# facebookresearch/vsc2022

Hardware: AMD Instinct MI355X
Metric: query-videos localized/sec @ 512-d SSCD (higher is better)
Workload: dtype fp32 results; int8 / fp16 MFMA pre-filters; 1 GPU; BASELINE configs[3]: full pipeline incl. score normalisation + TN localisation, 40000 query videos split over 1 GPU(s), 2000000 reference + 2000000 noise frames; query_videos_per_gpu=40000, query_frames_per_gpu=1000000, ref_frames=2000000, dim=512, global_k=48000000, candidates=1000000, pairs_localized=200000, matches=446939, hits=48000000, score_normalisation_in_step=True, parallelism=single GPU

## Files before the change

vsc2022_amd/csrc/tn.hip:

```cpp
#include <cfloat>

#include "kernels.h"

namespace vscmi {

typedef float f32x16 __attribute__((ext_vector_type(16)));
typedef float f32x4 __attribute__((ext_vector_type(4)));


template <class IDX>
struct TnStateT {
    int lq, lr, top, ms, n_nodes, sink, sink_q, sink_r;
    unsigned top_magic;
    float min_sim;
    const IDX* tidx;
    const float* tsim;
    const IDX* ilo;
    const IDX* ihi;
};

template <class IDX>
__device__ __forceinline__ int tn_div_top(const TnStateT<IDX>& g, int x) {
    return g.top == 1 ? x : (int)__umulhi((unsigned)x, g.top_magic);
}
template <class IDX>
__device__ __forceinline__ int tn_node_q(const TnStateT<IDX>& g, int v) { return v == 0 ? -1 : tn_div_top(g, v - 1); }
template <class IDX>
__device__ __forceinline__ int tn_node_k(const TnStateT<IDX>& g, int v) { return (v - 1) - tn_div_top(g, v - 1) * g.top; }
template <class IDX>
__device__ __forceinline__ int tn_node_r(const TnStateT<IDX>& g, int v) { return v == 0 ? -1 : g.tidx[v - 1]; }

template <class IDX>
__device__ __forceinline__ bool tn_edge_ok(const TnStateT<IDX>& g, int qi, int a, int d, int b) {
    const int qj = qi + d;
    const int ra = g.tidx[qi * g.top + a], rb = g.tidx[qj * g.top + b];
    const int rd = rb - ra;
    if (!(rd > 0 && rd < g.ms)) return false;
    const int lo = g.ilo[qi * g.ms + d], hi = g.ihi[qi * g.ms + d];
    if (lo <= hi && !(hi < ra || lo > rb)) return false;
    return g.tsim[qj * g.top + b] >= g.min_sim;
}

template <class IDX>
__device__ __forceinline__ bool tn_sink_ok(const TnStateT<IDX>& g, int u) {
    if (u == g.sink) return false;
    const int qu = tn_node_q(g, u), ru = tn_node_r(g, u);
    return g.sink_q > qu && g.sink_r > ru && g.sink_q - qu <= g.ms && g.sink_r - ru <= g.ms;
}

template <class IDX>
__device__ __forceinline__ int tn_edge_bit(const TnStateT<IDX>& g, int qi, int a, int d, int b) {
    return (((qi + d) * g.top + b) * g.ms + d) * g.top + a;
}

__device__ __forceinline__ unsigned long long first_max_key(float v, int o) {
    const float vz = v + 0.0f;
    const unsigned b = __float_as_uint(vz);
    unsigned hi = (b & 0x80000000u) ? ~b : (b | 0x80000000u);
    hi = (vz != vz) ? 1u : hi;
    const unsigned long long k = ((unsigned long long)hi << 32) | (unsigned)(0x7fffffff - o);
    return o < 0 ? 0ull : k;
}
__device__ __forceinline__ void first_max_unkey(unsigned long long k, float& v, int& o) {
    const unsigned hi = (unsigned)(k >> 32);
    const float kv = __uint_as_float((hi & 0x80000000u) ? (hi & 0x7fffffffu) : ~hi);
    v = k ? kv : 0.0f;
    o = k ? 0x7fffffff - (int)(unsigned)k : -1;
}
template <int FIRST_OFF>
__device__ __forceinline__ void first_max_reduce(float& v, int& o) {
    unsigned long long k = first_max_key(v, o);
#pragma unroll
    for (int off = FIRST_OFF; off >= 1; off >>= 1) {
        const unsigned long long ok = __shfl_xor(k, off);
        k = ok > k ? ok : k;
    }
    first_max_unkey(k, v, o);
}
__device__ __forceinline__ void wave_first_max(float& v, int& o) { first_max_reduce<32>(v, o); }
__device__ __forceinline__ void half_first_max(float& v, int& o) { first_max_reduce<16>(v, o); }


#ifdef VSC_TN_PROFILE
__device__ unsigned long long tn_prof[8];
#define TN_T0() unsigned long long t_prof = __builtin_readcyclecounter()
#define TN_T(k)                                                                          \
    do {                                                                                 \
        const unsigned long long t_now = __builtin_readcyclecounter();                   \
        if (threadIdx.x == 0) atomicAdd(&tn_prof[k], t_now - t_prof);                    \
        t_prof = t_now;                                                                  \
    } while (0)
#else
#define TN_T0() do {} while (0)
#define TN_T(k) do {} while (0)
#endif

template <class IDX, bool GSTATE>
__global__ __launch_bounds__(64) void tn_pair_kernel(TnPairArgs a) {
    extern __shared__ __attribute__((aligned(16))) char smem_lds[];
    char* const smem = GSTATE ? a.state + (int64_t)blockIdx.x * a.state_bytes : smem_lds;
    const int lane = threadIdx.x;
    if ((int)blockIdx.x >= a.n_work) return;
    const int pidx = a.work[blockIdx.x];
    int64_t qrow0 = 0, rrow0 = 0;
    int lq, lr;
    if (a.sims_in) {
        lq = a.sims_lq[pidx];
        lr = a.sims_lr[pidx];
    } else {
        const int qv = a.pair_q[pidx], rv = a.pair_r[pidx];
        qrow0 = a.q_off[qv];
        rrow0 = a.r_off[rv];
        lq = (int)(a.q_off[qv + 1] - qrow0);
        lr = (int)(a.r_off[rv + 1] - rrow0);
    }
    const int ms = a.prm.tn_max_step > 1 ? a.prm.tn_max_step : 1;
    const int top_cap = a.prm.tn_top_k;
    const int top = top_cap < lr ? top_cap : lr;
    int32_t* o_nbox = a.out_nbox + pidx;
    int32_t* o_boxes = a.out_boxes + (int64_t)pidx * VSC_TN_MAX_BOXES * 4;
    float* o_bmax = a.out_boxmax + (int64_t)pidx * VSC_TN_MAX_BOXES;
    if (lq <= 0 || top <= 0) {
        if (lane == 0) *o_nbox = 0;
        return;
    }
    const int n_nodes = 1 + lq * top;

    size_t off = 0;
    IDX* tidx = reinterpret_cast<IDX*>(smem + off);
    off += (size_t)a.max_lq * top_cap * sizeof(IDX);
    off = (off + 15) & ~(size_t)15;
    float* tsim = reinterpret_cast<float*>(smem + off);
    off += (size_t)a.max_lq * top_cap * 4;
    IDX* ilo = reinterpret_cast<IDX*>(smem + off);
    off += (size_t)a.max_lq * ms * sizeof(IDX);
    IDX* ihi = reinterpret_cast<IDX*>(smem + off);
    off += (size_t)a.max_lq * ms * sizeof(IDX);
    off = (off + 15) & ~(size_t)15;
    unsigned int* zero = reinterpret_cast<unsigned int*>(smem + off);
    const int zero_words = (lq * top * ms * top + 31) / 32;
    off += ((size_t)a.max_lq * top_cap * ms * top_cap + 31) / 32 * 4;
    off = (off + 15) & ~(size_t)15;
    float* dist = reinterpret_cast<float*>(smem + off);
    off += (size_t)(1 + a.max_lq * top_cap) * 4;
    IDX* par = reinterpret_cast<IDX*>(smem + off);
    off += (size_t)(1 + a.max_lq * top_cap) * sizeof(IDX);
    IDX* order = reinterpret_cast<IDX*>(smem + off);
    off += (size_t)(1 + a.max_lq * top_cap) * sizeof(IDX);
    IDX* indeg = reinterpret_cast<IDX*>(smem + off);
    off += (size_t)(1 + a.max_lq * top_cap) * sizeof(IDX);
    off = (off + 15) & ~(size_t)15;
    int* boxes = reinterpret_cast<int*>(smem + off);
    off += (size_t)VSC_TN_MAX_BOXES * 16;
    unsigned long long* okmask = reinterpret_cast<unsigned long long*>(smem + off);
    off += (size_t)a.max_lq * ((top_cap + 1) / 2) * 8;
    off = (off + 63) & ~(size_t)63;
    float* sims;
    if (a.sims_in) sims = const_cast<float*>(a.sims_in) + a.sims_off[pidx];
    else if ((int64_t)lq * lr <= a.lds_tile_floats) sims = reinterpret_cast<float*>(smem + off);
    else sims = a.slab + (int64_t)blockIdx.x * a.slab_floats;

    TN_T0();
    if (!a.sims_in) {
        const int hi = lane >> 5, l31 = lane & 31;
        const int nkg = a.dpad / 8;
        for (int qb = 0; qb < lq; qb += 32)
            for (int rb = 0; rb < lr; rb += 64) {
                const bool two = rb + 32 < lr;
                const float* ap = a.qfeat + (qrow0 + qb + l31) * a.dpad + hi * 4;
                const float* bp0 = a.rfeat + (rrow0 + rb + l31) * a.dpad + hi * 4;
                const float* bp1 = bp0 + (two ? 32 * (int64_t)a.dpad : 0);
                f32x16 acc0, acc1;
#pragma unroll
                for (int r = 0; r < 16; ++r) acc0[r] = acc1[r] = 0.0f;
                if (two) {
#pragma unroll 4
                    for (int g = 0; g < nkg; ++g) {
                        const f32x4 av = *reinterpret_cast<const f32x4*>(ap + g * 8);
                        const f32x4 bv0 = *reinterpret_cast<const f32x4*>(bp0 + g * 8);
                        const f32x4 bv1 = *reinterpret_cast<const f32x4*>(bp1 + g * 8);
#pragma unroll
                        for (int s = 0; s < 4; ++s) {
                            acc0 = __builtin_amdgcn_mfma_f32_32x32x2f32(av[s], bv0[s], acc0, 0, 0, 0);
                            acc1 = __builtin_amdgcn_mfma_f32_32x32x2f32(av[s], bv1[s], acc1, 0, 0, 0);
                        }
                    }
                } else {
#pragma unroll 4
                    for (int g = 0; g < nkg; ++g) {
                        const f32x4 av = *reinterpret_cast<const f32x4*>(ap + g * 8);
                        const f32x4 bv = *reinterpret_cast<const f32x4*>(bp0 + g * 8);
#pragma unroll
                        for (int s = 0; s < 4; ++s)
                            acc0 = __builtin_amdgcn_mfma_f32_32x32x2f32(av[s], bv[s], acc0, 0, 0, 0);
                    }
                }
#pragma unroll
                for (int r = 0; r < 16; ++r) {
                    const int q = qb + (r & 3) + 8 * (r >> 2) + 4 * hi;
                    const int rr = rb + l31;
                    if (q < lq && rr < lr) sims[(int64_t)q * lr + rr] = acc0[r] + a.bias;
                    if (two && q < lq && rr + 32 < lr) sims[(int64_t)q * lr + rr + 32] = acc1[r] + a.bias;
                }
            }
    }
    for (int x = lane; x < zero_words; x += 64) zero[x] = 0;
    __threadfence_block();
    __syncthreads();
    TN_T(0);

    if (top_cap <= 8 && (lq >= 16 || lr <= 128)) {
        for (int q0 = 0; q0 < lq; q0 += 64) {
            const int q = q0 + lane;
            float ts[8];
            int ti[8];
#pragma unroll
            for (int e = 0; e < 8; ++e) {
                ts[e] = -INFINITY;
                ti[e] = -1;
            }
            if (q < lq) {
                const float* row = sims + (int64_t)q * lr;
                for (int r = 0; r < lr; ++r) {
                    const float sv = row[r];
                    if (!(sv > ts[7]) && ti[7] >= 0) continue;
#pragma unroll
                    for (int e = 7; e >= 1; --e) {
                        const bool empty_above = ti[e - 1] < 0;
                        const bool up = empty_above || sv > ts[e - 1];
                        const bool here = !up && (ti[e] < 0 || sv > ts[e]);
                        ts[e] = up ? ts[e - 1] : (here ? sv : ts[e]);
                        ti[e] = up ? ti[e - 1] : (here ? r : ti[e]);
                    }
                    if (ti[0] < 0 || sv > ts[0]) {
                        ts[0] = sv;
                        ti[0] = r;
                    }
                }
#pragma unroll
                for (int e = 0; e < 8; ++e)
                    if (e < top) {
                        tidx[q * top + e] = (IDX)ti[e];
                        tsim[q * top + e] = ts[e];
                    }
            }
        }
    } else {
        for (int q = 0; q < lq; ++q) {
            const float* row = sims + (int64_t)q * lr;
            float prev_s = INFINITY;
            int prev_r = -1;
            for (int e = 0; e < top; ++e) {
                float bs = 0.0f;
                int br = -1;
                for (int r = lane; r < lr; r += 64) {
                    const float s = row[r];
                    const bool after = (s < prev_s) || (s == prev_s && r > prev_r);
                    if (after && (br < 0 || s > bs)) {
                        bs = s;
                        br = r;
                    }
                }
                wave_first_max(bs, br);
                if (lane == 0) {
                    tidx[q * top + e] = (IDX)br;
                    tsim[q * top + e] = bs;
                }
                prev_s = bs;
                prev_r = br;
            }
        }
    }
    __syncthreads();

    TnStateT<IDX> g;
    g.lq = lq; g.lr = lr; g.top = top; g.ms = ms; g.n_nodes = n_nodes; g.sink = n_nodes - 1;
    g.sink_q = lq - 1;
    g.sink_r = tidx[(lq - 1) * top + top - 1];
    g.min_sim = a.prm.min_sim;
    g.top_magic = (unsigned)((0x100000000ull + (unsigned)top - 1u) / (unsigned)top);
    g.tidx = tidx; g.tsim = tsim; g.ilo = ilo; g.ihi = ihi;

    for (int qi = lane; qi < lq; qi += 64) {
        int lo = 1, hi = 0;
        for (int d = 1; d < ms; ++d) {
            ilo[qi * ms + d] = (IDX)lo;
            ihi[qi * ms + d] = (IDX)hi;
            if (qi + d >= lq) continue;
            int nlo = lo, nhi = hi;
            for (int b = 0; b < top; ++b) {
                bool any = false;
                for (int aa = 0; aa < top && !any; ++aa) any = tn_edge_ok(g, qi, aa, d, b);
                if (any) {
                    const int rb = tidx[(qi + d) * top + b];
                    if (nlo > nhi) nlo = nhi = rb;
                    else {
                        nlo = rb < nlo ? rb : nlo;
                        nhi = rb > nhi ? rb : nhi;
                    }
                }
            }
            lo = nlo;
            hi = nhi;
        }
    }
    __syncthreads();

    TN_T(1);
    const int P = (ms - 1) * top;
    int nbox = 0;
    bool have_order = false;
    const int hw_half = lane >> 5, hw_o = lane & 31;
    const int hw_d = ms - 1 - hw_o / top, hw_aa = hw_o % top;
    const int hw_bit_off = hw_d * top + hw_aa + hw_half * ms * top;
    const int hw_pred_off = 1 + hw_aa - hw_d * top;
    for (int it = 0; it <= a.prm.max_path; ++it) {
        if (lane == 0) {
            dist[0] = 0.0f;
            par[0] = 0;
        }
        __syncthreads();
        for (int qj = 0; qj < lq; ++qj) {
            int b_first = 0;
            if (P <= 32) {
                const int half = hw_half, o = hw_o, d = hw_d, aa = hw_aa;
                const int qi = qj - d;
                const int pred = qj * top + hw_pred_off;
                for (int b0 = 0; b0 < top; b0 += 2) {
                    const int b = b0 + half;
                    const int v = 1 + qj * top + b;
                    const bool mine = b < top && v != g.sink;
                    float c = 0.0f;
                    int oo = -1;
                    const int mslot = qj * ((top + 1) / 2) + (b0 >> 1);
                    bool ok;
                    if (it == 0) {
                        ok = mine && o < P && qi >= 0 && tn_edge_ok(g, qi, aa, d, b);
                        const unsigned long long m = __ballot(ok);
                        if (lane == 0) okmask[mslot] = m;
                    } else {
                        ok = (okmask[mslot] >> lane) & 1ull;
                    }
                    if (ok) {
                        const int bit = (qj * top + b0) * ms * top + hw_bit_off;
                        const bool z = (zero[bit >> 5] >> (bit & 31)) & 1u;
                        const float w = z ? 0.0f : tsim[qj * top + b];
                        c = dist[pred] + w;
                        oo = o;
                    }
                    half_first_max(c, oo);
                    const int pw = __shfl(pred, (lane & 32) | (oo < 0 ? 0 : oo));
                    if (mine && o == 0) {
                        if (oo < 0 || !(c >= 0.0f)) {
                            dist[v] = 0.0f;
                            par[v] = (IDX)v;
                        } else {
                            dist[v] = c;
                            par[v] = (IDX)pw;
                        }
                    }
                }
                b_first = (qj == lq - 1) ? top - 1 : top;
            }
            if (qj == lq - 1) TN_T(2);
            for (int b = b_first; b < top; ++b) {
                const int v = 1 + qj * top + b;
                const bool is_sink = (v == g.sink);
                float best = 0.0f;
                int arg = -1;
                for (int o0 = 0; o0 < P; o0 += 64) {
                    const int o = o0 + lane;
                    float c = 0.0f;
                    int oo = -1;
                    if (o < P) {
                        const int d = ms - 1 - o / top, aa = o % top;
                        const int qi = qj - d;
                        if (qi >= 0 && tn_edge_ok(g, qi, aa, d, b)) {
                            const int bit = tn_edge_bit(g, qi, aa, d, b);
                            const bool z = (zero[bit >> 5] >> (bit & 31)) & 1u;
                            const float w = (z || is_sink) ? 0.0f : tsim[qj * top + b];
                            c = dist[1 + qi * top + aa] + w;
                            oo = o;
                        }
                    }
                    wave_first_max(c, oo);
                    if (oo >= 0 && (arg < 0 || c > best)) {
                        best = c;
                        arg = oo;
                    }
                }
                int arg_node = -1;
                if (arg >= 0) arg_node = 1 + (qj - (ms - 1 - arg / top)) * top + arg % top;
                if (is_sink) {
                    for (int u0 = 0; u0 < n_nodes - 1; u0 += 64) {
                        const int u = u0 + lane;
                        float c = 0.0f;
                        int oo = -1;
                        if (u < n_nodes - 1 && tn_sink_ok(g, u)) {
                            bool regular = false;
                            if (u != 0) {
                                const int qi = tn_node_q(g, u), aa = tn_node_k(g, u);
                                const int d = qj - qi;
                                if (d >= 1 && d < ms) regular = tn_edge_ok(g, qi, aa, d, b);
                            }
                            if (!regular) {
                                c = dist[u] + 0.0f;
                                oo = u;
                            }
                        }
                        wave_first_max(c, oo);
                        if (oo >= 0 && (arg_node < 0 || c > best)) {
                            best = c;
                            arg_node = oo;
                        }
                    }
                }
                if (lane == 0) {
                    if (arg_node < 0 || !(best >= 0.0f)) {
                        dist[v] = 0.0f;
                        par[v] = (IDX)v;
                    } else {
                        dist[v] = best;
                        par[v] = (IDX)arg_node;
                    }
                }
            }
            __syncthreads();
        }

        TN_T(3);
        float mx = -FLT_MAX;
        int mxn = -1;
        for (int v = lane; v < n_nodes; v += 64) {
            const float dv = dist[v];
            if (mxn < 0 || dv > mx) {
                mx = dv;
                mxn = v;
            }
        }
        wave_first_max(mx, mxn);
        int ties = 0;
        for (int v = lane; v < n_nodes; v += 64) ties += (dist[v] == mx) ? 1 : 0;
#pragma unroll
        for (int off2 = 32; off2 >= 1; off2 >>= 1) ties += __shfl_xor(ties, off2);
        int vend = mxn;
        if (!(mx > 0.0f)) {
            vend = 0;
        } else if (ties > 1) {
            if (!have_order) {
                for (int v = lane; v < n_nodes; v += 64) {
                    int deg = 0;
                    if (v != 0) {
                        const int qj = tn_node_q(g, v), b = tn_node_k(g, v);
                        for (int d = 1; d < ms; ++d) {
                            const int qi = qj - d;
                            if (qi < 0) break;
                            for (int aa = 0; aa < top; ++aa) deg += tn_edge_ok(g, qi, aa, d, b) ? 1 : 0;
                        }
                        if (v == g.sink) {
                            for (int u = 0; u < n_nodes - 1; ++u) {
                                if (!tn_sink_ok(g, u)) continue;
                                bool regular = false;
                                if (u != 0) {
                                    const int qi = tn_node_q(g, u), aa = tn_node_k(g, u);
                                    const int d = qj - qi;
                                    if (d >= 1 && d < ms) regular = tn_edge_ok(g, qi, aa, d, b);
                                }
                                deg += regular ? 0 : 1;
                            }
                        }
                    }
                    indeg[v] = (IDX)deg;
                }
                __syncthreads();
                if (lane == 0) {
                    int head = 0, tail = 0;
                    for (int v = 0; v < n_nodes; ++v)
                        if (indeg[v] == 0) order[tail++] = (IDX)v;
                    while (head < tail) {
                        const int u = order[head++];
                        bool to_sink_regular = false;
                        if (u != 0) {
                            const int qi = tn_node_q(g, u), aa = tn_node_k(g, u);
                            for (int d = 1; d < ms && qi + d < lq; ++d)
                                for (int b = 0; b < top; ++b)
                                    if (tn_edge_ok(g, qi, aa, d, b)) {
                                        const int v = 1 + (qi + d) * top + b;
                                        if (v == g.sink) to_sink_regular = true;
                                        if (--indeg[v] == 0) order[tail++] = (IDX)v;
                                    }
                        }
                        if (!to_sink_regular && tn_sink_ok(g, u))
                            if (--indeg[g.sink] == 0) order[tail++] = (IDX)g.sink;
                    }
                }
                have_order = true;
                __syncthreads();
            }
            int bestpos = 0x7fffffff;
            for (int t = lane; t < n_nodes; t += 64)
                if (dist[order[t]] == mx && t < bestpos) bestpos = t;
#pragma unroll
            for (int off2 = 32; off2 >= 1; off2 >>= 1) {
                const int o2 = __shfl_xor(bestpos, off2);
                bestpos = o2 < bestpos ? o2 : bestpos;
            }
            vend = order[bestpos];
        }

        TN_T(4);
        int accepted = 0, stop = 0;
        int bq0 = 0, br0 = 0, bq1 = 0, br1 = 0;
        if (lane == 0) {
            int cnt = 0;
            for (int v = vend;;) {
                const int u = par[v];
                if (v != 0 && v != g.sink) ++cnt;
                if (u == v) break;
                if (u != 0) {
                    const int qi = tn_node_q(g, u), aa = tn_node_k(g, u);
                    const int qj = tn_node_q(g, v), b = tn_node_k(g, v);
                    const int d = qj - qi;
                    if (d >= 1 && d < ms && tn_edge_ok(g, qi, aa, d, b)) {
                        const int bit = tn_edge_bit(g, qi, aa, d, b);
                        zero[bit >> 5] |= 1u << (bit & 31);
                    }
                }
                v = u;
            }
            if (cnt == 0) {
                stop = 1;
            } else {
                int plen = 0;
                for (int v = vend;;) {
                    indeg[plen++] = (IDX)v;
                    if (par[v] == v) break;
                    v = par[v];
                }
                float score = 0.0f;
                int qmin = 0, qmax = 0, rmin = 0, rmax = 0, c2 = 0;
                for (int x = plen - 1; x >= 0; --x) {
                    const int v = indeg[x];
                    if (v == 0 || v == g.sink) continue;
                    const int q = tn_node_q(g, v), r = tn_node_r(g, v);
                    score += tsim[v - 1];
                    if (c2 == 0) {
                        qmin = qmax = q;
                        rmin = rmax = r;
                    } else {
                        qmin = q < qmin ? q : qmin;
                        qmax = q > qmax ? q : qmax;
                        rmin = r < rmin ? r : rmin;
                        rmax = r > rmax ? r : rmax;
                    }
                    ++c2;
                }
                if (!(score > 0.0f)) qmin = qmax = rmin = rmax = 0;
                const int dq = qmax - qmin, dr = rmax - rmin;
                const float ave = __fdiv_rn((float)(dr + dq), 2.0f);
                bool ok = (ave != 0.0f) && (__fdiv_rn(score, ave) > a.prm.min_sim) &&
                          ((dr < dq ? dr : dq) > a.prm.min_length);
                if (ok && nbox > 0) {
                    float mxi = -INFINITY;
                    for (int kx = 0; kx < nbox; ++kx) {
                        const int* o = boxes + 4 * kx;
                        const float lt0 = (float)(qmin > o[0] ? qmin : o[0]);
                        const float lt1 = (float)(rmin > o[1] ? rmin : o[1]);
                        const float rb0 = (float)(qmax < o[2] ? qmax : o[2]);
                        const float rb1 = (float)(rmax < o[3] ? rmax : o[3]);
                        const float w = rb0 - lt0 > 0.0f ? rb0 - lt0 : 0.0f;
                        const float h = rb1 - lt1 > 0.0f ? rb1 - lt1 : 0.0f;
                        const float inter = __fmul_rn(w, h);
                        const float aa2 = __fmul_rn((float)dq, (float)dr);
                        const float ab = __fmul_rn((float)(o[2] - o[0]), (float)(o[3] - o[1]));
                        const float iou = __fdiv_rn(inter, __fsub_rn(__fadd_rn(aa2, ab), inter));
                        mxi = iou > mxi ? iou : mxi;
                    }
                    ok = mxi < a.prm.max_iou;
                }
                if (ok && nbox < VSC_TN_MAX_BOXES) {
                    boxes[4 * nbox + 0] = qmin;
                    boxes[4 * nbox + 1] = rmin;
                    boxes[4 * nbox + 2] = qmax;
                    boxes[4 * nbox + 3] = rmax;
                    accepted = 1;
                    bq0 = qmin; br0 = rmin; bq1 = qmax; br1 = rmax;
                }
            }
        }
        stop = __shfl(stop, 0);
        accepted = __shfl(accepted, 0);
        __syncthreads();
        TN_T(5);
        if (stop) break;
        if (accepted) {
            bq0 = __shfl(bq0, 0); br0 = __shfl(br0, 0); bq1 = __shfl(bq1, 0); br1 = __shfl(br1, 0);
            float m = -INFINITY;
            const int w = br1 - br0, h = bq1 - bq0;
            for (int y = 0; y < h; ++y) {
                const float* srow = sims + (int64_t)(bq0 + y) * lr + br0;
                for (int x = lane; x < w; x += 64) {
                    const float s = srow[x];
                    m = s > m ? s : m;
                }
            }
#pragma unroll
            for (int off2 = 32; off2 >= 1; off2 >>= 1) {
                const float o2 = __shfl_xor(m, off2);
                m = o2 > m ? o2 : m;
            }
            if (lane == 0) {
                o_boxes[4 * nbox + 0] = bq0;
                o_boxes[4 * nbox + 1] = br0;
                o_boxes[4 * nbox + 2] = bq1;
                o_boxes[4 * nbox + 3] = br1;
                o_bmax[nbox] = __fsub_rn(m, a.bias);
            }
            ++nbox;
        }
        TN_T(6);
    }
    if (lane == 0) *o_nbox = nbox;
}

#ifdef VSC_TN_PROFILE
extern "C" int vsc_tn_prof_read(unsigned long long* out8, int reset) {
    if (hipMemcpyFromSymbol(out8, HIP_SYMBOL(tn_prof), sizeof(tn_prof)) != hipSuccess) return -1;
    if (reset) {
        unsigned long long z[8] = {};
        if (hipMemcpyToSymbol(HIP_SYMBOL(tn_prof), z, sizeof(z)) != hipSuccess) return -1;
    }
    return 0;
}
#endif

size_t tn_state_bytes_host(int max_lq, int top_cap, int ms, int idx_bytes) {
    const size_t n_nodes = 1 + (size_t)max_lq * top_cap;
    const size_t ib = (size_t)idx_bytes;
    size_t b = 0;
    b += (size_t)max_lq * top_cap * ib;
    b = (b + 15) & ~(size_t)15;
    b += (size_t)max_lq * top_cap * 4;
    b += (size_t)max_lq * ms * ib * 2;
    b = (b + 15) & ~(size_t)15;
    b += ((size_t)max_lq * top_cap * ms * top_cap + 31) / 32 * 4;
    b = (b + 15) & ~(size_t)15;
    b += n_nodes * 4;
    b += n_nodes * ib * 3;
    b = (b + 15) & ~(size_t)15;
    b += (size_t)VSC_TN_MAX_BOXES * 16;
    b += (size_t)max_lq * ((top_cap + 1) / 2) * 8;
    b = (b + 63) & ~(size_t)63;
    return b;
}

int launch_tn_pairs(const TnPairArgs& a, size_t lds_bytes, hipStream_t stream) {
    if (a.n_work <= 0) return VSC_OK;
    static PerDeviceOnce once;
    if (a.state) {
        hipLaunchKernelGGL((tn_pair_kernel<int, true>), dim3((unsigned)a.n_work), dim3(64), 0, stream, a);
        VSC_HIP(hipGetLastError());
        return VSC_OK;
    }
    if (once.first()) {
        VSC_HIP(hipFuncSetAttribute(reinterpret_cast<const void*>(&tn_pair_kernel<short, false>),
                                    hipFuncAttributeMaxDynamicSharedMemorySize, 158 * 1024));
        once.commit();
    }
    hipLaunchKernelGGL((tn_pair_kernel<short, false>), dim3((unsigned)a.n_work), dim3(64), lds_bytes, stream, a);
    VSC_HIP(hipGetLastError());
    return VSC_OK;
}


__global__ __launch_bounds__(64) void tn_sims_kernel(TnSimsArgs a) {
    const int lane = threadIdx.x, hi = lane >> 5, l31 = lane & 31;
    const int qb = blockIdx.y * 32, rb = blockIdx.x * 32;
    const float* ap = a.qfeat + (a.qrow0 + qb + l31) * a.dpad + hi * 4;
    const float* bp = a.rfeat + (a.rrow0 + rb + l31) * a.dpad + hi * 4;
    f32x16 acc;
#pragma unroll
    for (int r = 0; r < 16; ++r) acc[r] = 0.0f;
    const int nkg = a.dpad / 8;
#pragma unroll 4
    for (int g = 0; g < nkg; ++g) {
        const f32x4 av = *reinterpret_cast<const f32x4*>(ap + g * 8);
        const f32x4 bv = *reinterpret_cast<const f32x4*>(bp + g * 8);
#pragma unroll
        for (int s = 0; s < 4; ++s) acc = __builtin_amdgcn_mfma_f32_32x32x2f32(av[s], bv[s], acc, 0, 0, 0);
    }
#pragma unroll
    for (int r = 0; r < 16; ++r) {
        const int q = qb + (r & 3) + 8 * (r >> 2) + 4 * hi;
        const int rr = rb + l31;
        if (q < a.lq && rr < a.lr) a.out[(int64_t)q * a.lr + rr] = acc[r] + a.bias;
    }
}

int launch_tn_sims(const TnSimsArgs& a, hipStream_t stream) {
    if (a.lq <= 0 || a.lr <= 0) return VSC_OK;
    hipLaunchKernelGGL(tn_sims_kernel, dim3((a.lr + 31) / 32, (a.lq + 31) / 32), dim3(64), 0, stream, a);
    VSC_HIP(hipGetLastError());
    return VSC_OK;
}

}
```

Baseline: 20240 query-videos/s.

## Restructure TN DP row pass into lane groups with DPP max reduction

Replaces the half-wave per-node relaxation in the temporal-network longest-path DP with a grouped scheme. Each lane group of 8 or 16 handles one target node, and every lane folds several predecessor steps serially before a DPP-based two-stage 32-bit max reduction. The 64-bit shuffle reduction is removed and the path also covers P>32 when the step count is at most 6. The cost is more okmask LDS slots, extra template instantiations and register pressure. Tie-breaking on first-max ordering has to be preserved exactly.

```diff
diff --git a/vsc2022_amd/csrc/tn.hip b/vsc2022_amd/csrc/tn.hip
--- a/vsc2022_amd/csrc/tn.hip
+++ b/vsc2022_amd/csrc/tn.hip
@@ -1,4 +1,5 @@
 #include <cfloat>
+#include <type_traits>
 
 #include "kernels.h"
 
@@ -53,12 +54,15 @@
     return (((qi + d) * g.top + b) * g.ms + d) * g.top + a;
 }
 
-__device__ __forceinline__ unsigned long long first_max_key(float v, int o) {
+
+__device__ __forceinline__ unsigned first_max_key_hi(float v) {
     const float vz = v + 0.0f;
     const unsigned b = __float_as_uint(vz);
-    unsigned hi = (b & 0x80000000u) ? ~b : (b | 0x80000000u);
-    hi = (vz != vz) ? 1u : hi;
-    const unsigned long long k = ((unsigned long long)hi << 32) | (unsigned)(0x7fffffff - o);
+    const unsigned hi = b ^ ((unsigned)((int)b >> 31) | 0x80000000u);
+    return (vz != vz) ? 1u : hi;
+}
+__device__ __forceinline__ unsigned long long first_max_key(float v, int o) {
+    const unsigned long long k = ((unsigned long long)first_max_key_hi(v) << 32) | (unsigned)(0x7fffffff - o);
     return o < 0 ? 0ull : k;
 }
 __device__ __forceinline__ void first_max_unkey(unsigned long long k, float& v, int& o) {
@@ -78,7 +82,39 @@
     first_max_unkey(k, v, o);
 }
 __device__ __forceinline__ void wave_first_max(float& v, int& o) { first_max_reduce<32>(v, o); }
-__device__ __forceinline__ void half_first_max(float& v, int& o) { first_max_reduce<16>(v, o); }
+
+template <int CTRL>
+__device__ __forceinline__ unsigned dpp_u32(unsigned x) {
+    return (unsigned)__builtin_amdgcn_update_dpp(0, (int)x, CTRL, 0xf, 0xf, true);
+}
+__device__ __forceinline__ unsigned umax32(unsigned a, unsigned b) { return a > b ? a : b; }
+__device__ __forceinline__ unsigned group_max_u32(unsigned x, bool g16) {
+    x = umax32(x, dpp_u32<0xB1>(x));
+    x = umax32(x, dpp_u32<0x4E>(x));
+    x = umax32(x, dpp_u32<0x141>(x));
+    if (g16) x = umax32(x, dpp_u32<0x140>(x));
+    return x;
+}
+__device__ __forceinline__ unsigned long long group_first_max_key(unsigned hi, unsigned lo, bool g16) {
+    const unsigned m = group_max_u32(hi, g16);
+    const unsigned l = group_max_u32(hi == m ? lo : 0u, g16);
+    return ((unsigned long long)m << 32) | l;
+}
+
+constexpr int TN_ROW_SMAX = 6;
+__host__ __device__ __forceinline__ int tn_row_group(int top) { return top <= 4 ? 16 : 8; }
+__host__ __device__ __forceinline__ int tn_row_steps(int top, int ms) {
+    const int G = tn_row_group(top);
+    return ((ms - 1) * top + G - 1) / G;
+}
+__host__ __device__ __forceinline__ int tn_row_passes(int top) {
+    const int n_grp = 64 / tn_row_group(top);
+    return (top + n_grp - 1) / n_grp;
+}
+__host__ __device__ __forceinline__ int tn_row_mask_slots(int top_cap, int ms) {
+    const int S = tn_row_steps(top_cap, ms);
+    return tn_row_passes(top_cap) * (S < TN_ROW_SMAX ? S : TN_ROW_SMAX);
+}
 
 
 #ifdef VSC_TN_PROFILE
@@ -153,7 +189,7 @@
     int* boxes = reinterpret_cast<int*>(smem + off);
     off += (size_t)VSC_TN_MAX_BOXES * 16;
     unsigned long long* okmask = reinterpret_cast<unsigned long long*>(smem + off);
-    off += (size_t)a.max_lq * ((top_cap + 1) / 2) * 8;
+    off += (size_t)a.max_lq * tn_row_mask_slots(top_cap, ms) * 8;
     off = (off + 63) & ~(size_t)63;
     float* sims;
     if (a.sims_in) sims = const_cast<float*>(a.sims_in) + a.sims_off[pidx];
@@ -310,10 +346,80 @@
     const int P = (ms - 1) * top;
     int nbox = 0;
     bool have_order = false;
-    const int hw_half = lane >> 5, hw_o = lane & 31;
-    const int hw_d = ms - 1 - hw_o / top, hw_aa = hw_o % top;
-    const int hw_bit_off = hw_d * top + hw_aa + hw_half * ms * top;
-    const int hw_pred_off = 1 + hw_aa - hw_d * top;
+    const int rp_G = tn_row_group(top), rp_S = tn_row_steps(top, ms), rp_np = tn_row_passes(top);
+    const int rp_ngrp = 64 / rp_G;
+    const bool row_pass = rp_S <= TN_ROW_SMAX;
+    const int rp_g = lane & (rp_G - 1), rp_grp = lane / rp_G;
+    int rp_d[TN_ROW_SMAX];
+    int rp_bit_off[TN_ROW_SMAX];
+#pragma unroll
+    for (int s = 0; s < TN_ROW_SMAX; ++s) {
+        const int o = rp_g + s * rp_G;
+        const int od = tn_div_top(g, o);
+        const int d = ms - 1 - od, aa = o - od * top;
+        rp_d[s] = o < P ? d : 0x3fffffff;
+        rp_bit_off[s] = d * top + aa + rp_grp * ms * top;
+    }
+    auto row_pass_fn = [&](auto first_c, auto ns_c, int qj) {
+        constexpr bool FIRST = decltype(first_c)::value;
+        constexpr int NS = decltype(ns_c)::value;
+        const int pred0 = qj * top + 1 - P + rp_g;
+        for (int p = 0; p < rp_np; ++p) {
+            const int b = p * rp_ngrp + rp_grp;
+            const int v = 1 + qj * top + b;
+            const bool mine = b < top && v != g.sink;
+            const int bit0 = (qj * top + p * rp_ngrp) * ms * top;
+            unsigned long long* const mrow = okmask + ((size_t)qj * rp_np + p) * rp_S;
+            unsigned long long mk[TN_ROW_SMAX];
+            if (!FIRST) {
+#pragma unroll
+                for (int s = 0; s < NS; ++s) mk[s] = mrow[s];
+            }
+            const float wv = mine ? tsim[v - 1] : 0.0f;
+            unsigned hi = 0u;
+            int sb = 0;
+#pragma unroll
+            for (int s = 0; s < TN_ROW_SMAX; ++s) {
+                if (s >= (NS ? NS : rp_S)) break;
+                const int pred = pred0 + s * rp_G;
+                const int bit = bit0 + rp_bit_off[s];
+                unsigned hs = 0u;
+                if (FIRST) {
+                    const int d = rp_d[s], qi = qj - d;
+                    const bool ok = mine && qi >= 0 && tn_edge_ok(g, qi, pred - 1 - qi * top, d, b);
+                    const unsigned long long m = __ballot(ok);
+                    if (lane == 0) mrow[s] = m;
+                    if (ok) {
+                        const bool z = __builtin_amdgcn_ubfe(zero[bit >> 5], (unsigned)bit, 1u);
+                        hs = first_max_key_hi(dist[pred] + (z ? 0.0f : wv));
+                    }
+                } else {
+                    const bool ok = (mk[s] >> lane) & 1ull;
+                    const int pi = ok ? pred : 0, bi = ok ? bit : 0;
+                    const bool z = __builtin_amdgcn_ubfe(zero[bi >> 5], (unsigned)bi, 1u);
+                    hs = first_max_key_hi(dist[pi] + (z ? 0.0f : wv));
+                    hs = ok ? hs : 0u;
+                }
+                const bool gt = hs > hi;
+                hi = gt ? hs : hi;
+                sb = gt ? s : sb;
+            }
+            const unsigned lo = hi ? (unsigned)(0x7fffffff - (rp_g + sb * rp_G)) : 0u;
+            const unsigned long long k = group_first_max_key(hi, lo, rp_G == 16);
+            float c;
+            int oo;
+            first_max_unkey(k, c, oo);
+            if (mine && rp_g == 0) {
+                if (oo < 0 || !(c >= 0.0f)) {
+                    dist[v] = 0.0f;
+                    par[v] = (IDX)v;
+                } else {
+                    dist[v] = c;
+                    par[v] = (IDX)(qj * top + 1 - P + oo);
+                }
+            }
+        }
+    };
     for (int it = 0; it <= a.prm.max_path; ++it) {
         if (lane == 0) {
             dist[0] = 0.0f;
@@ -322,43 +428,17 @@
         __syncthreads();
         for (int qj = 0; qj < lq; ++qj) {
             int b_first = 0;
-            if (P <= 32) {
-                const int half = hw_half, o = hw_o, d = hw_d, aa = hw_aa;
-                const int qi = qj - d;
-                const int pred = qj * top + hw_pred_off;
-                for (int b0 = 0; b0 < top; b0 += 2) {
-                    const int b = b0 + half;
-                    const int v = 1 + qj * top + b;
-                    const bool mine = b < top && v != g.sink;
-                    float c = 0.0f;
-                    int oo = -1;
-                    const int mslot = qj * ((top + 1) / 2) + (b0 >> 1);
-                    bool ok;
-                    if (it == 0) {
-                        ok = mine && o < P && qi >= 0 && tn_edge_ok(g, qi, aa, d, b);
-                        const unsigned long long m = __ballot(ok);
-                        if (lane == 0) okmask[mslot] = m;
-                    } else {
-                        ok = (okmask[mslot] >> lane) & 1ull;
-                    }
-                    if (ok) {
-                        const int bit = (qj * top + b0) * ms * top + hw_bit_off;
-                        const bool z = (zero[bit >> 5] >> (bit & 31)) & 1u;
-                        const float w = z ? 0.0f : tsim[qj * top + b];
-                        c = dist[pred] + w;
-                        oo = o;
-                    }
-                    half_first_max(c, oo);
-                    const int pw = __shfl(pred, (lane & 32) | (oo < 0 ? 0 : oo));
-                    if (mine && o == 0) {
-                        if (oo < 0 || !(c >= 0.0f)) {
-                            dist[v] = 0.0f;
-                            par[v] = (IDX)v;
-                        } else {
-                            dist[v] = c;
-                            par[v] = (IDX)pw;
-                        }
-                    }
+            if (row_pass) {
+                using std::integral_constant;
+                if (it == 0) row_pass_fn(std::true_type{}, integral_constant<int, 0>{}, qj);
+                else switch (rp_S) {
+                    case 1: row_pass_fn(std::false_type{}, integral_constant<int, 1>{}, qj); break;
+                    case 2: row_pass_fn(std::false_type{}, integral_constant<int, 2>{}, qj); break;
+                    case 3: row_pass_fn(std::false_type{}, integral_constant<int, 3>{}, qj); break;
+                    case 4: row_pass_fn(std::false_type{}, integral_constant<int, 4>{}, qj); break;
+                    case 5: row_pass_fn(std::false_type{}, integral_constant<int, 5>{}, qj); break;
+                    case 6: row_pass_fn(std::false_type{}, integral_constant<int, 6>{}, qj); break;
+                    default: row_pass_fn(std::false_type{}, integral_constant<int, 0>{}, qj); break;
                 }
                 b_first = (qj == lq - 1) ? top - 1 : top;
             }
@@ -649,7 +729,7 @@
     b += n_nodes * ib * 3;
     b = (b + 15) & ~(size_t)15;
     b += (size_t)VSC_TN_MAX_BOXES * 16;
-    b += (size_t)max_lq * ((top_cap + 1) / 2) * 8;
+    b += (size_t)max_lq * tn_row_mask_slots(top_cap, ms) * 8;
     b = (b + 63) & ~(size_t)63;
     return b;
 }
```

After: 20370 query-videos/s (median of 6 runs). About the same (+0.7%).
